# returaj/gan_mpc

Hardware: AMD Instinct MI355X
Metric: trajectories/sec (rollout+backward+critic step) at batch=1024, H=50 (higher is better)
Workload: dtype f32

## Files before the change

### gan_mpc_amd/csrc/gmpc_api_solve.hip

```cpp
#include "gmpc_ctx.h"
#include "gmpc_fused_solve.h"

static TrajArgs base_traj(gmpc_ctx* c, int B, const float* goal) {
  TrajArgs a;
  memset(&a, 0, sizeof(a));
  a.B = B; a.n = c->sh.n; a.m = c->sh.m; a.T = c->sh.T;
  a.dyn = c->dyn; a.cost = c->cost; a.mpc_w = c->mpc_w; a.goal = goal;
  return a;
}

static DynlTrajArgs base_dynl(gmpc_ctx* c, int B, const float* goal) {
  DynlTrajArgs a;
  memset(&a, 0, sizeof(a));
  a.B = B; a.T = c->sh.T; a.d = c->dl; a.cost = c->cost; a.mpc_w = c->mpc_w; a.goal = goal;
  return a;
}

extern "C" int gmpc_rollout_cost(gmpc_ctx* c, int B, const float* x0, const float* U,
                                 const float* goal, float* X, float* costs, void* stream) {
  TRY(check_call(c, B));
  if (!x0 || !U || !goal || !X) return fail(GMPC_EINVAL, "null argument");
  hipStream_t s = static_cast<hipStream_t>(stream);
  c->solB = 0;
  c->gradB = 0;
  if (c->dynl) {
    DynlTrajArgs d = base_dynl(c, B, goal);
    d.x0 = x0; d.U = U; d.X = X; d.costs = costs; d.obj = c->obj;
    {
      ProfScope ps(c, PROF_ROLLOUT, s);
      gmpc_launch_dynl_rollout(d, s);
    }
    HIP_TRY(hipGetLastError());
    return 0;
  }
  TrajArgs a = base_traj(c, B, goal);
  a.x0 = x0; a.U = U; a.X = X; a.costs = costs; a.obj = c->obj; a.masks = c->masks;
  {
    ProfScope ps(c, PROF_ROLLOUT, s);
    gmpc_launch_rollout(a, s);
  }
  HIP_TRY(hipGetLastError());
  return 0;
}

static int backward_pass(gmpc_ctx* c, int B, const float* X, const float* U, const float* goal,
                         const int* active, float* K, float* k, float* grad, float* adj, float* AB,
                         int* cont, const gmpc_ilqr_opts* opts, hipStream_t s) {
  const gmpc_shape& sh = c->sh;
  if (c->big) {
    if (c->lin_event) HIP_TRY(hipEventRecord(c->lin_event, s));
    if (gmpc_launch_terminal(B, sh.T, sh.n, c->cost, c->mpc_w, X, active, c->QT, c->qT, s) != 0)
      return fail(GMPC_EINVAL, "terminal: unsupported fout");
    HIP_TRY(hipGetLastError());
    {
      ProfScope ps(c, PROF_RICCATI, s);
      if (gmpc_big_backward(c->bw, B, c->dyn, c->lp, c->masks, X, U, goal, c->mpc_w, c->QT, c->qT, active,
                            c->Ks, k, grad ? grad : c->grads, adj ? adj : c->adjs, nullptr, nullptr, s,
                            c->dynl ? &c->dl : nullptr) != 0)
        return fail(GMPC_EINVAL, "large-state backward: Jacobian kernel does not cover this shape");
      if (K != c->Ks)
        HIP_TRY(hipMemcpyAsync(K, c->Ks, (size_t)B * sh.T * sh.m * sh.n * sizeof(float),
                               hipMemcpyDeviceToDevice, s));
    }
    if (cont)
      gmpc_launch_big_cont(B, sh.T, sh.m, U, c->bw.gn2, c->iters, c->obj, c->alpha, c->obj_step,
                           c->U_step, *opts, active, cont, s);
    HIP_TRY(hipGetLastError());
    return 0;
  }
  {
    ProfScope ps(c, PROF_TERMINAL, s);
    if (gmpc_launch_terminal(B, sh.T, sh.n, c->cost, c->mpc_w, X, active, c->QT, c->qT, s) != 0)
      return fail(GMPC_EINVAL, "terminal: unsupported fout");
  }
  {
    ProfScope ps(c, PROF_LINEARIZE, s);
    const char* lin_env = getenv("GMPC_LIN");
    const bool lin_dense = lin_env != nullptr && strcmp(lin_env, "dense") == 0;
    if (c->dynl) {
      gmpc_launch_dynl_jac(B, sh.T, sh.T, 0, c->dl, X, U, active, AB, s);
      c->lin_kernel = "k_dynl_jac";
    } else if (!lin_dense && gmpc_launch_linearize_sparse(B * sh.T, sh.T, sh.n, sh.m, c->dyn, c->lp, c->masks,
                                                          active, AB, 1, 0, s) == 0) {
      c->lin_kernel = sh.n > 16 ? "k_linearize_sparse (rows 0..15) + k_linearize_regs (rows 16..n-1)"
                                : "k_linearize_sparse";
    } else if (gmpc_launch_linearize_regs(B * sh.T, sh.T, sh.n, sh.m, c->dyn, c->lp, c->masks, active, AB, 1, 0,
                                          s) == 0) {
      snprintf(c->lin_kernel_buf, sizeof(c->lin_kernel_buf), "%s", gmpc_linearize_regs_last_name());
      c->lin_kernel = c->lin_kernel_buf;
    } else if (gmpc_launch_linearize_mfma(B * sh.T, sh.T, sh.n, sh.m, c->dyn, c->lp, c->masks, active, AB, 1, 0,
                                          s) != 0) {
      if (gmpc_launch_linearize(B, sh.T, sh.n, sh.m, c->dyn, c->masks, active, AB, s) != 0)
        return fail(GMPC_EINVAL, "linearize: unsupported row count for n=%d", sh.n);
      c->lin_kernel = "k_linearize (vector ALU)";
    } else {
      c->lin_kernel = "k_linearize_mfma";
    }
  }
  HIP_TRY(hipGetLastError());
  if (c->lin_event) HIP_TRY(hipEventRecord(c->lin_event, s));
  RiccatiArgs r;
  memset(&r, 0, sizeof(r));
  r.B = B; r.n = sh.n; r.ng = c->nx; r.m = sh.m; r.T = sh.T; r.mode = 0;
  r.X = X; r.U = U; r.goal = goal; r.mpc_w = c->mpc_w; r.AB = AB; r.QT = c->QT; r.qT = c->qT;
  r.active = active; r.K = K; r.k = k; r.grad = grad; r.adj = adj;
  if (cont) {
    r.cont = cont; r.iters = c->iters; r.obj = c->obj; r.alpha = c->alpha;
    r.obj_step = c->obj_step; r.U_step = c->U_step; r.opts = *opts;
  }
  {
    ProfScope ps(c, PROF_RICCATI, s);
    gmpc_launch_riccati(r, s);
  }
  HIP_TRY(hipGetLastError());
  return 0;
}

extern "C" int gmpc_lqr_backward(gmpc_ctx* c, int B, const float* X, const float* U,
                                 const float* goal, float* K, float* k, float* grad,
                                 float* adjoints, float* AB, void* stream) {
  TRY(check_call(c, B));
  if (!X || !U || !goal) return fail(GMPC_EINVAL, "null argument");
  hipStream_t s = static_cast<hipStream_t>(stream);
  if (c->big && AB) return fail(GMPC_EINVAL, "AB output is not materialised for n > 64 (pass NULL)");
  c->solB = 0;
  c->gradB = 0;
  if (!c->dynl) gmpc_launch_masks(B, c->sh.n, c->sh.m, c->sh.T, c->dyn, X, U, c->masks, s);
  return backward_pass(c, B, X, U, goal, nullptr, K ? K : c->Ks, k ? k : c->ks, grad, adjoints,
                       AB ? AB : c->AB, nullptr, nullptr, s);
}

extern "C" int gmpc_lqr_backward_after_rollout(gmpc_ctx* c, int B, const float* X, const float* U,
                                               const float* goal, float* K, float* k, float* grad,
                                               float* adjoints, float* AB, void* stream) {
  TRY(check_call(c, B));
  if (!X || !U || !goal) return fail(GMPC_EINVAL, "null argument");
  if (c->big && AB) return fail(GMPC_EINVAL, "AB output is not materialised for n > 64 (pass NULL)");
  hipStream_t s = static_cast<hipStream_t>(stream);
  c->solB = 0;
  c->gradB = 0;
  return backward_pass(c, B, X, U, goal, nullptr, K ? K : c->Ks, k ? k : c->ks, grad, adjoints,
                       AB ? AB : c->AB, nullptr, nullptr, s);
}

static void dynl_ls_eval(void* user, const TrajArgs& t, int max_items, hipStream_t s) {
  gmpc_ctx* c = static_cast<gmpc_ctx*>(user);
  DynlTrajArgs d = base_dynl(c, t.B, t.goal);
  d.item_b = t.item_b; d.item_k = t.item_k; d.nitems = t.nitems;
  d.Xn = t.X; d.Un = t.Uio; d.Kg = t.Kg; d.kg = t.kg;
  d.Xc = t.Xc; d.Uc = t.Uc; d.objc = t.objc; d.alpha_0 = t.alpha_0;
  gmpc_launch_dynl_candidates(d, max_items, s);
}

extern "C" int gmpc_ilqr_solve(gmpc_ctx* c, int B, const float* x0, const float* U_init,
                               const float* goal, const gmpc_ilqr_opts* opts, float* X, float* U,
                               float* obj, float* grad, float* adjoints, int* iterations,
                               void* stream) {
  TRY(check_call(c, B));
  if (!x0 || !U_init || !goal || !opts) return fail(GMPC_EINVAL, "null argument");
  if (opts->make_psd) return fail(GMPC_EINVAL, "make_psd=1 is not on the reference path");
  hipStream_t s = static_cast<hipStream_t>(stream);
  c->solB = 0;
  c->solBox = false;
  c->gradB = 0;
  const gmpc_shape& sh = c->sh;
  const size_t n = sh.n, m = sh.m, T = sh.T;
  HIP_TRY(hipMemcpyAsync(c->Us, U_init, B * T * m * sizeof(float), hipMemcpyDeviceToDevice, s));
  HIP_TRY(hipMemcpyAsync(c->goals, goal, B * (T + 1) * (size_t)c->nx * sizeof(float), hipMemcpyDeviceToDevice, s));
  HIP_TRY(hipMemsetAsync(c->iters, 0, B * sizeof(int), s));
  std::vector<float> init(3 * (size_t)B);
  for (int b = 0; b < B; ++b) {
    init[b] = opts->alpha_0;
    init[B + b] = INFINITY;
    init[2 * (size_t)B + b] = INFINITY;
  }
  HIP_TRY(hipMemcpyAsync(c->alpha, init.data(), B * sizeof(float), hipMemcpyHostToDevice, s));
  HIP_TRY(hipMemcpyAsync(c->obj_step, init.data() + B, B * sizeof(float), hipMemcpyHostToDevice, s));
  HIP_TRY(hipMemcpyAsync(c->U_step, init.data() + 2 * (size_t)B, B * sizeof(float),
                         hipMemcpyHostToDevice, s));
  HIP_TRY(hipStreamSynchronize(s));
  if (c->dynl) {
    DynlTrajArgs d = base_dynl(c, B, c->goals);
    d.x0 = x0; d.U = c->Us; d.X = c->Xs; d.costs = nullptr; d.obj = c->obj;
    gmpc_launch_dynl_rollout(d, s);
  } else {
    TrajArgs a = base_traj(c, B, c->goals);
    a.x0 = x0; a.U = c->Us; a.X = c->Xs; a.costs = nullptr; a.obj = c->obj; a.masks = c->masks;
    gmpc_launch_rollout(a, s);
  }
  TRY(backward_pass(c, B, c->Xs, c->Us, c->goals, nullptr, c->Ks, c->ks, c->grads, c->adjs, c->AB,
                    c->cont, opts, s));
  TrajArgs ls = base_traj(c, B, c->goals);
  ls.X = c->Xs; ls.Uio = c->Us; ls.obj = c->obj; ls.masks = c->masks; ls.Kg = c->Ks; ls.kg = c->ks;
  ls.Xc = c->Xc; ls.Uc = c->Uc; ls.maskc = c->maskc; ls.active = c->cont; ls.alpha = c->alpha;
  ls.obj_step = c->obj_step; ls.U_step = c->U_step; ls.iters = c->iters;
  ls.alpha_0 = opts->alpha_0; ls.alpha_min = opts->alpha_min;
  LsPlan plan;
  if (gmpc_ls_plan(ls, c->ncu, c->dynl, &plan) != 0 && opts->maxiter > 0)
    return fail(GMPC_EINVAL, "line search: alpha_0 / alpha_min need more than %d rounds", GMPC_LS_ROUNDS_MAX);
  HIP_TRY(hipMemsetAsync(c->lsw.prevk, 0, B * sizeof(int), s));
  HIP_TRY(hipMemsetAsync(c->lsw.counts + GMPC_LS_ROUNDS_MAX, 0, (1 + GMPC_LS_STATS) * sizeof(int), s));
  if (!c->hcont) {
    HIP_TRY(hipHostMalloc(reinterpret_cast<void**>(&c->hcont), (size_t)GMPC_POLL_DEPTH * c->maxB * sizeof(int),
                          hipHostMallocDefault));
    for (int i = 0; i < GMPC_POLL_DEPTH; ++i) HIP_TRY(hipEventCreateWithFlags(&c->poll_ev[i], hipEventDisableTiming));
  }
  for (int it = 0; it < opts->maxiter; ++it) {
    const int slot = it % GMPC_POLL_DEPTH;
    int* hc = c->hcont + (size_t)slot * c->maxB;
    if (it >= GMPC_POLL_DEPTH) {
      HIP_TRY(hipEventSynchronize(c->poll_ev[slot]));
      bool any = false;
      for (int b = 0; b < B; ++b) any |= hc[b] != 0;
      if (!any) break;
    }
    HIP_TRY(hipMemcpyAsync(hc, c->cont, B * sizeof(int), hipMemcpyDeviceToHost, s));
    HIP_TRY(hipEventRecord(c->poll_ev[slot], s));
    {
      ProfScope ps(c, PROF_LINESEARCH, s);
      gmpc_launch_linesearch(ls, plan, c->lsw, s, c->dynl ? &dynl_ls_eval : nullptr, c);
    }
    TRY(backward_pass(c, B, c->Xs, c->Us, c->goals, c->cont, c->Ks, c->ks, c->grads, c->adjs, c->AB,
                      c->cont, opts, s));
  }
  if (X) HIP_TRY(hipMemcpyAsync(X, c->Xs, B * (T + 1) * n * sizeof(float), hipMemcpyDeviceToDevice, s));
  if (U) HIP_TRY(hipMemcpyAsync(U, c->Us, B * T * m * sizeof(float), hipMemcpyDeviceToDevice, s));
  if (obj) HIP_TRY(hipMemcpyAsync(obj, c->obj, B * sizeof(float), hipMemcpyDeviceToDevice, s));
  if (grad) HIP_TRY(hipMemcpyAsync(grad, c->grads, B * T * m * sizeof(float), hipMemcpyDeviceToDevice, s));
  if (adjoints)
    HIP_TRY(hipMemcpyAsync(adjoints, c->adjs, B * (T + 1) * n * sizeof(float), hipMemcpyDeviceToDevice, s));
  if (iterations)
    HIP_TRY(hipMemcpyAsync(iterations, c->iters, B * sizeof(int), hipMemcpyDeviceToDevice, s));
  HIP_TRY(hipStreamSynchronize(s));
  c->solB = B;
  return 0;
}

static int solve_one_launch(gmpc_ctx* c, int B, const float* x0, const float* U_init, const float* goal,
                            const gmpc_ilqr_opts* opts, float* X, float* U, float* obj, float* grad, float* adjoints,
                            int* iterations, void* stream, const char* who, bool box, const float* u_lo,
                            const float* u_hi) {
  TRY(check_call(c, B));
  if (!x0 || !U_init || !goal || !opts) return fail(GMPC_EINVAL, "null argument");
  if (opts->make_psd) return fail(GMPC_EINVAL, "make_psd=1 is not on the reference path");
  const gmpc_shape& sh = c->sh;
  if (c->dynl) return fail(GMPC_EINVAL, "%s: MLP dynamics only (dyn_lstm_features = %d)", who, sh.dyn_lstm_features);
  if (c->big)
    return fail(GMPC_EINVAL, "%s: n <= 64 and m <= 32 only (n=%d m=%d)", who, sh.n, sh.m);
  if (sh.T > GMPC_FZ_MAX_T) return fail(GMPC_EINVAL, "%s: T <= %d only (T=%d)", who, GMPC_FZ_MAX_T, sh.T);
  const int k_max = gmpc_ls_halvings(opts->alpha_0, opts->alpha_min, GMPC_FZ_MAX_HALVINGS + 1);
  if (k_max > GMPC_FZ_MAX_HALVINGS)
    return fail(GMPC_EINVAL, "%s: alpha_0 / alpha_min allow more than %d halvings", who, GMPC_FZ_MAX_HALVINGS);
  hipStream_t s = static_cast<hipStream_t>(stream);
  c->solB = 0;
  c->solBox = false;
  c->gradB = 0;
  FusedSolveArgs a;
  memset(&a, 0, sizeof(a));
  a.n = sh.n; a.m = sh.m; a.T = sh.T; a.k_max = k_max;
  a.dyn = c->dyn; a.cost = c->cost; a.mpc_w = c->mpc_w; a.opts = *opts;
  a.x0 = x0; a.U_init = U_init; a.goal_in = goal;
  a.X = c->Xs; a.U = c->Us; a.goal = c->goals; a.AB = c->AB; a.QT = c->QT; a.qT = c->qT;
  a.K = c->Ks; a.k = c->ks; a.grad = c->grads; a.adj = c->adjs;
  a.obj = c->obj; a.alpha = c->alpha; a.obj_step = c->obj_step; a.U_step = c->U_step; a.iters = c->iters;
  a.cand = c->fzcand;
  a.oX = X; a.oU = U; a.oobj = obj; a.ograd = grad; a.oadj = adjoints; a.oiters = iterations;
  if (box) {
    BoxSolveArgs x;
    x.u_lo = u_lo; x.u_hi = u_hi;
    x.count = c->box_count; x.iters = c->box_iters; x.clamped = c->box_clamped;
    gmpc_launch_ilqr_box(a, x, B, s);
  } else {
    gmpc_launch_ilqr_fused(a, B, s);
  }
  HIP_TRY(hipGetLastError());
  return 0;
}

extern "C" int gmpc_ilqr_solve_fused(gmpc_ctx* c, int B, const float* x0, const float* U_init,
                                     const float* goal, const gmpc_ilqr_opts* opts, float* X, float* U,
                                     float* obj, float* grad, float* adjoints, int* iterations,
                                     void* stream) {
  TRY(solve_one_launch(c, B, x0, U_init, goal, opts, X, U, obj, grad, adjoints, iterations, stream, "fused solve",
                       false, nullptr, nullptr));
  c->solB = B;
  return 0;
}

extern "C" int gmpc_ilqr_solve_box(gmpc_ctx* c, int B, const float* x0, const float* U_init,
                                   const float* goal, const gmpc_ilqr_opts* opts, float* X, float* U,
                                   float* obj, float* grad, float* adjoints, int* iterations,
                                   void* stream, const float* u_lo, const float* u_hi) {
  return solve_one_launch(c, B, x0, U_init, goal, opts, X, U, obj, grad, adjoints, iterations, stream, "box solve",
                          true, u_lo, u_hi);
}

extern "C" int gmpc_ilqr_solve_box_held(gmpc_ctx* c, int B, const float* x0, const float* U_init,
                                        const float* goal, const gmpc_ilqr_opts* opts, float* X, float* U,
                                        float* obj, float* grad, float* adjoints, int* iterations,
                                        void* stream, const float* u_lo, const float* u_hi) {
  TRY(solve_one_launch(c, B, x0, U_init, goal, opts, X, U, obj, grad, adjoints, iterations, stream, "box solve",
                       true, u_lo, u_hi));
  gmpc_launch_box_clamped(B, c->sh.T, c->sh.m, c->Us, c->grads, u_lo, u_hi, c->box_mask,
                          static_cast<hipStream_t>(stream));
  HIP_TRY(hipGetLastError());
  c->solB = B;
  c->solBox = true;
  return 0;
}

extern "C" int gmpc_cem_solve(gmpc_ctx* c, int B, const float* x0, const float* goal, const float* u_lo,
                              const float* u_hi, const gmpc_cem_opts* o, float* mean_io, float* std_io, float* X,
                              float* obj, float* costs, int* elites, float* samples, void* stream) {
  TRY(check_call(c, B));
  const gmpc_shape& sh = c->sh;
  if (c->dynl) return fail(GMPC_EINVAL, "cem: MLP dynamics only (dyn_lstm_features = %d)", sh.dyn_lstm_features);
  for (int l = 0; l <= sh.dyn_layers; ++l)
    if (sh.dyn_dims[l] > 256) return fail(GMPC_EINVAL, "cem: dynamics width %d above 256", sh.dyn_dims[l]);
  for (int l = 0; l <= sh.cost_layers; ++l)
    if (sh.cost_dims[l] > 256) return fail(GMPC_EINVAL, "cem: cost width %d above 256", sh.cost_dims[l]);
  if (sh.n + sh.m > 256) return fail(GMPC_EINVAL, "cem: n + m = %d above 256", sh.n + sh.m);
  if (!o) return fail(GMPC_EINVAL, "cem: opts is null");
  if (!x0 || !goal || !mean_io || !std_io) return fail(GMPC_EINVAL, "cem: x0, goal, mean_io and std_io must not be null");
  if (o->num_samples < 1 || o->num_samples > 4096)
    return fail(GMPC_EINVAL, "cem: num_samples = %d outside [1, 4096]", o->num_samples);
  if (o->num_elites < 1 || o->num_elites > o->num_samples)
    return fail(GMPC_EINVAL, "cem: num_elites = %d outside [1, num_samples = %d]", o->num_elites, o->num_samples);
  if (o->max_iter < 0) return fail(GMPC_EINVAL, "cem: max_iter = %d is negative", o->max_iter);
  if (!(o->sampling_smoothing >= 0.f && o->sampling_smoothing < 1.f))
    return fail(GMPC_EINVAL, "cem: sampling_smoothing = %g outside [0, 1)", (double)o->sampling_smoothing);
  if (!(o->evolution_smoothing >= 0.f && o->evolution_smoothing <= 1.f))
    return fail(GMPC_EINVAL, "cem: evolution_smoothing = %g outside [0, 1]", (double)o->evolution_smoothing);
  hipStream_t s = static_cast<hipStream_t>(stream);
  const int N = o->num_samples;
  float* cost_buf = costs;
  if (!cost_buf && o->max_iter > 0) {
    TRY(c->cw.aux.grow(c, (size_t)B * N));
    cost_buf = c->cw.aux.p;
  }
  CemRollArgs r;
  memset(&r, 0, sizeof(r));
  r.B = B; r.N = N; r.T = sh.T; r.n = sh.n; r.m = sh.m;
  r.dyn = c->dyn; r.cost = c->cost; r.mpc_w = c->mpc_w;
  r.x0 = x0; r.goal = goal; r.mean = mean_io; r.sd = std_io; r.lo = u_lo; r.hi = u_hi;
  r.rng.key0 = (uint32_t)(o->seed & 0xFFFFFFFFull); r.rng.key1 = (uint32_t)(o->seed >> 32);
  r.rng.beta = o->sampling_smoothing;
  r.rng.cbeta = sqrtf(1.f - r.rng.beta * r.rng.beta);
  r.costs = cost_buf;
  CemUpdArgs u;
  memset(&u, 0, sizeof(u));
  u.B = B; u.N = N; u.E = o->num_elites; u.T = sh.T; u.m = sh.m;
  u.costs = cost_buf; u.lo = u_lo; u.hi = u_hi; u.mean = mean_io; u.sd = std_io;
  u.gamma = o->evolution_smoothing;
  for (int i = 0; i < o->max_iter; ++i) {
    const bool last = i == o->max_iter - 1;
    r.rng.it = (uint32_t)(o->iter_offset + i);
    r.samples = last ? samples : nullptr;
    u.rng = r.rng;
    u.elites = last ? elites : nullptr;
    if (gmpc_launch_cem_rollout(r, s) || gmpc_launch_cem_update(u, s)) return fail(GMPC_EINVAL, "cem: shape not covered");
  }
  if (X || obj) {
    if (!obj) {
      TRY(c->cw.aux2.grow(c, (size_t)B));
      obj = c->cw.aux2.p;
    }
    r.N = 1; r.mean_row = 1; r.samples = nullptr; r.costs = obj; r.X = X;
    if (gmpc_launch_cem_rollout(r, s)) return fail(GMPC_EINVAL, "cem: shape not covered");
  }
  HIP_TRY(hipGetLastError());
  return 0;
}


extern "C" int gmpc_get_cost(gmpc_ctx* c, int B, const float* x, const float* u, const float* goal_row,
                             int terminal, float* cost, void* stream) {
  TRY(check_call(c, B));
  if (!x || !cost || (!terminal && (!u || !goal_row))) return fail(GMPC_EINVAL, "null argument");
  gmpc_launch_get_cost(B, c->sh.n, c->nx, c->sh.m, c->cost, c->mpc_w, x, u, goal_row, terminal != 0, cost,
                       static_cast<hipStream_t>(stream));
  HIP_TRY(hipGetLastError());
  return 0;
}

extern "C" int gmpc_predict(gmpc_ctx* c, int B, const float* x, const float* u, float* next_x,
                            void* stream) {
  TRY(check_call(c, B));
  if (!x || !u || !next_x) return fail(GMPC_EINVAL, "null argument");
  hipStream_t s = static_cast<hipStream_t>(stream);
  const size_t n = c->sh.n;
  c->solB = 0;
  c->gradB = 0;
  HIP_TRY(hipMemsetAsync(c->goals, 0, (size_t)B * 2 * n * sizeof(float), s));
  if (c->dynl) {
    DynlTrajArgs d = base_dynl(c, B, c->goals);
    d.T = 1;
    d.x0 = x; d.U = u; d.X = c->Xc; d.costs = nullptr; d.obj = c->obj;
    gmpc_launch_dynl_rollout(d, s);
  } else {
    TrajArgs a = base_traj(c, B, c->goals);
    a.T = 1;
    a.x0 = x; a.U = u; a.X = c->Xc; a.costs = nullptr; a.obj = c->obj; a.masks = c->masks;
    gmpc_launch_rollout(a, s);
  }
  HIP_TRY(hipGetLastError());
  HIP_TRY(hipMemcpy2DAsync(next_x, n * sizeof(float), c->Xc + n, 2 * n * sizeof(float), n * sizeof(float),
                           B, hipMemcpyDeviceToDevice, s));
  return 0;
}

extern "C" long gmpc_linesearch_candidates(gmpc_ctx* c) {
  if (!c) return -1;
  int v = 0;
  if (hipSetDevice(c->device) != hipSuccess || hipDeviceSynchronize() != hipSuccess ||
      hipMemcpy(&v, c->lsw.counts + GMPC_LS_ROUNDS_MAX, sizeof(int), hipMemcpyDeviceToHost) != hipSuccess)
    return -1;
  return v;
}

extern "C" int gmpc_linesearch_stats(gmpc_ctx* c, long* out, int n) {
  if (!c || !out) return fail(GMPC_EINVAL, "ctx / out is null");
  int v[GMPC_LS_STATS];
  HIP_TRY(hipSetDevice(c->device));
  HIP_TRY(hipDeviceSynchronize());
  HIP_TRY(hipMemcpy(v, c->lsw.counts + GMPC_LS_ROUNDS_MAX + 1, sizeof(v), hipMemcpyDeviceToHost));
  for (int i = 0; i < n; ++i) out[i] = i < GMPC_LS_STATS ? v[i] : 0;
  return 0;
}
```

### gan_mpc_amd/csrc/gmpc_linearize_sparse.hip

```cpp
#include <cstdio>
#include <type_traits>

#include "gmpc_launch.h"

typedef float f32x4 __attribute__((ext_vector_type(4)));
typedef unsigned v4u __attribute__((ext_vector_type(4)));
typedef unsigned v2u __attribute__((ext_vector_type(2)));

#define GMPC_LIN_PADROWS 24
#define GMPC_SP_H 200
#define GMPC_SP_Z 200
#define GMPC_SP_STR 220
#define GMPC_SP_CAP 216
#define GMPC_SP_WAVE_BYTES (16 * GMPC_SP_STR * 4 + 3 * GMPC_SP_CAP * 4)
#define GMPC_SP_RD 3
#define GMPC_SP_ROW 256

static bool sparse_form(int L, const int* dims, int n, int m) {
  const int Lh = L - 1;
  if (Lh < 2 || n + m > 32 || n < 1) return false;
  for (int l = 1; l <= Lh; ++l)
    if (dims[l] != GMPC_SP_H) return false;
  return true;
}

__global__ void k_pack_sparse(const float* W, float* dst) {
  const int e = blockIdx.x * blockDim.x + threadIdx.x;
  if (e >= GMPC_SP_H * GMPC_SP_H) return;
  const int i = e / GMPC_SP_H, o = e - i * GMPC_SP_H;
  const int t = i >> 4;
  const int slot = i < 192 ? 64 * (t >> 2) + 4 * (i & 15) + (t & 3) : i;
  dst[(size_t)o * GMPC_SP_ROW + slot] = W[e];
}

size_t gmpc_linsparse_floats(int L, const int* dims, int n, int m) {
  if (!sparse_form(L, dims, n, m)) return 0;
  return (size_t)(L - 2) * (GMPC_SP_H + GMPC_LIN_PADROWS) * GMPC_SP_ROW + GMPC_SP_ROW;
}

void gmpc_linsparse_prepare(const MlpDesc& dyn, int n, int m, float* p, LinPad* out, hipStream_t s) {
  for (int l = 0; l < GMPC_MAX_LAYERS; ++l) out->WSP[l] = nullptr;
  if (!sparse_form(dyn.L, dyn.dims, n, m)) return;
  p = reinterpret_cast<float*>((reinterpret_cast<uintptr_t>(p) + 1023) & ~(uintptr_t)1023);
  for (int l = 1; l < dyn.L - 1; ++l) {
    out->WSP[l] = p;
    hipLaunchKernelGGL(k_pack_sparse, dim3((GMPC_SP_H * GMPC_SP_H + 255) / 256), dim3(256), 0, s, dyn.W[l], p);
    p += (size_t)(GMPC_SP_H + GMPC_LIN_PADROWS) * GMPC_SP_ROW;
  }
}

__global__ __launch_bounds__(GMPC_THREADS, 2) void k_linearize_sparse(
    int NSamp, int T, int n, int m, int Lh, LinPad lp, const uint32_t* masks, const int* active, float* AB,
    int samp_mul, int samp_add) {
  extern __shared__ __attribute__((aligned(16))) char smem[];
  const int lane = threadIdx.x & 63, wave = __builtin_amdgcn_readfirstlane(threadIdx.x >> 6);
  const int g = lane >> 4, l16 = lane & 15;
  const int nm = n + m;
  const int nrow = n < 16 ? n : 16;
  char* wbase = smem + wave * GMPC_SP_WAVE_BYTES;
  float* st = reinterpret_cast<float*>(wbase);
  unsigned* lk = reinterpret_cast<unsigned*>(wbase + 16 * GMPC_SP_STR * 4);
  unsigned* lt = lk + GMPC_SP_CAP;
  if (lane < 16 * 8) st[(lane >> 3) * GMPC_SP_STR + GMPC_SP_H + (lane & 7)] = 0.f;
  if (lane + 64 < 16 * 8) st[((lane + 64) >> 3) * GMPC_SP_STR + GMPC_SP_H + (lane & 7)] = 0.f;

  const int lw = l16 * 16, lwt = (192 + (l16 & 7)) * 4;
  const int ls = l16 * GMPC_SP_STR * 4;
  const int tsel = l16 >= 8 ? 1 : 0;
  const unsigned* lkl = lk + g;
  const unsigned* ltl_ = lt + 2 * g + tsel;
  const int lsn = l16 < n ? l16 * 4 : (1 << 28);
  const __amdgpu_buffer_rsrc_t rsl = __builtin_amdgcn_make_buffer_rsrc(
      const_cast<float*>(lp.WLP), 0, (GMPC_SP_H + GMPC_LIN_PADROWS) * n * (int)sizeof(float), 0x00020000);
  const __amdgpu_buffer_rsrc_t rs0 = __builtin_amdgcn_make_buffer_rsrc(
      const_cast<float*>(lp.WTP[0]), 0, (GMPC_SP_H + GMPC_LIN_PADROWS) * 32 * (int)sizeof(float), 0x00020000);

  constexpr int WPB = GMPC_THREADS / 64;
  for (int s = blockIdx.x * WPB + wave; s < NSamp; s += gridDim.x * WPB) {
    const size_t sid = (size_t)s * samp_mul + samp_add;
    if (active != nullptr && active[sid / T] == 0) continue;
    const uint32_t* mrow = masks + sid * Lh * GMPC_MW;

    auto build = [&](int ml) -> int {
      __builtin_amdgcn_wave_barrier();
      int base = 0;
#pragma unroll
      for (int c = 0; c < 4; ++c) {
        const uint32_t lo = __builtin_amdgcn_readfirstlane(mrow[ml * GMPC_MW + 2 * c]);
        uint32_t hi = c < 3 ? __builtin_amdgcn_readfirstlane(mrow[ml * GMPC_MW + 2 * c + 1]) : 0u;
        const uint32_t lo_m = c < 3 ? lo : (lo & 0xFFu);
        const uint32_t word = lane < 32 ? lo_m : hi;
        const int pos = base + (int)__builtin_amdgcn_mbcnt_hi(hi, __builtin_amdgcn_mbcnt_lo(lo_m, 0u));
        const unsigned u = 64 * c + lane;
        if ((word >> (lane & 31)) & 1u) {
          const bool odd = (u & 1u) != 0;
          lk[pos] = u;
          *reinterpret_cast<v2u*>(lt + 2 * pos) = v2u{odd ? GMPC_SP_Z : u, odd ? u : GMPC_SP_Z};
        }
        base += __builtin_popcount(lo_m) + __builtin_popcount(hi);
      }
      if (lane < 16) {
        lk[base + lane] = GMPC_SP_Z;
        *reinterpret_cast<v2u*>(lt + 2 * (base + lane)) = v2u{GMPC_SP_Z, GMPC_SP_Z};
      }
      __builtin_amdgcn_wave_barrier();
      return base;
    };

    auto layer = [&](int l, auto seedc) __attribute__((always_inline)) {
      constexpr bool seed = decltype(seedc)::value;
      const int np = (build(l) + 3) >> 2;
      const __amdgpu_buffer_rsrc_t wrs = __builtin_amdgcn_make_buffer_rsrc(
          const_cast<float*>(lp.WSP[l]), 0, (GMPC_SP_H + GMPC_LIN_PADROWS) * GMPC_SP_ROW * 4, 0x00020000);
      f32x4 acc[13];
      struct Ops { float w[13]; float b; unsigned k, kt; };
      Ops r[GMPC_SP_RD];
      auto tables = [&](Ops& o, int p) {
        o.k = lkl[4 * p];
        o.kt = ltl_[8 * p];
      };
      auto loads = [&](Ops& o) {
        const int k = (int)o.k, kt = (int)o.kt;
        const int vo = (k << 10) + lw, vt = (kt << 10) + lwt;
#pragma unroll
        for (int q = 0; q < 3; ++q) {
          const v4u a = __builtin_amdgcn_raw_buffer_load_b128(wrs, vo + 256 * q, 0, 0);
          o.w[4 * q] = __uint_as_float(a.x); o.w[4 * q + 1] = __uint_as_float(a.y);
          o.w[4 * q + 2] = __uint_as_float(a.z); o.w[4 * q + 3] = __uint_as_float(a.w);
        }
        o.w[12] = __uint_as_float(__builtin_amdgcn_raw_buffer_load_b32(wrs, vt, 0, 0));
        if constexpr (seed) o.b = __uint_as_float(__builtin_amdgcn_raw_buffer_load_b32(rsl, k * n * 4 + lsn, 0, 0));
        else o.b = st[(ls >> 2) + k];
      };
      auto step = [&](int p, Ops& cur, Ops& ahead2) __attribute__((always_inline)) {
        loads(ahead2);
        tables(cur, p + 3);
        __builtin_amdgcn_sched_barrier(0);
#pragma unroll
        for (int t = 0; t < 13; ++t) acc[t] = __builtin_amdgcn_mfma_f32_16x16x4f32(cur.w[t], cur.b, acc[t], 0, 0, 0);
        __builtin_amdgcn_sched_barrier(0);
      };
      if (np == 0) {
#pragma unroll
        for (int t = 0; t < 13; ++t) acc[t] = f32x4{0.f, 0.f, 0.f, 0.f};
      } else {
        tables(r[0], 0); tables(r[1], 1); tables(r[2], 2);
        loads(r[0]); loads(r[1]);
        loads(r[2]);
        tables(r[0], 3);
        __builtin_amdgcn_sched_barrier(0);
#pragma unroll
        for (int t = 0; t < 13; ++t)
          acc[t] = __builtin_amdgcn_mfma_f32_16x16x4f32(r[0].w[t], r[0].b, f32x4{0.f, 0.f, 0.f, 0.f}, 0, 0, 0);
        __builtin_amdgcn_sched_barrier(0);
        int p = 1;
        for (; p + 3 <= np; p += 3) {
          step(p, r[1], r[0]);
          step(p + 1, r[2], r[1]);
          step(p + 2, r[0], r[2]);
        }
        if (p < np) step(p, r[1], r[0]);
        if (p + 1 < np) step(p + 1, r[2], r[1]);
      }
      mfma_fence<false>(acc[0], acc[1], acc[2], acc[3], acc[4], acc[5], acc[6], acc[7], acc[8], acc[9], acc[10],
                        acc[11], acc[12]);
      __builtin_amdgcn_wave_barrier();
      float* srow = st + l16 * GMPC_SP_STR;
#pragma unroll
      for (int t = 0; t < 12; ++t)
        *reinterpret_cast<f32x4*>(srow + 32 * (t >> 1) + 16 * (t & 1) + 4 * g) = acc[t];
      *reinterpret_cast<f32x4*>(srow + (g < 2 ? 192 : 200) + 4 * g) = acc[12];
      __builtin_amdgcn_wave_barrier();
      if (g < 2) {
        const f32x4 x = *reinterpret_cast<const f32x4*>(srow + 192 + 4 * g);
        const f32x4 y = *reinterpret_cast<const f32x4*>(srow + 208 + 4 * g);
        *reinterpret_cast<f32x4*>(srow + 192 + 4 * g) = x + y;
      }
      __builtin_amdgcn_wave_barrier();
    };
    layer(Lh - 1, std::true_type{});
    for (int l = Lh - 2; l >= 1; --l) layer(l, std::false_type{});

    {
      const int np = (build(0) + 3) >> 2;
      f32x4 acc0 = {0.f, 0.f, 0.f, 0.f}, acc1 = {0.f, 0.f, 0.f, 0.f};
      const bool two = nm > 16;
      struct Ops0 { float w0, w1, b; unsigned k; };
      Ops0 r[GMPC_SP_RD];
      auto tables = [&](Ops0& o, int p) { o.k = lkl[4 * p]; };
      auto loads = [&](Ops0& o) {
        const int vo = (int)(o.k << 7) + l16 * 4;
        o.w0 = __uint_as_float(__builtin_amdgcn_raw_buffer_load_b32(rs0, vo, 0, 0));
        o.w1 = __uint_as_float(__builtin_amdgcn_raw_buffer_load_b32(rs0, vo + 64, 0, 0));
        o.b = st[(ls >> 2) + o.k];
      };
      auto step = [&](int p, Ops0& cur, Ops0& ahead2) __attribute__((always_inline)) {
        loads(ahead2);
        tables(cur, p + 3);
        __builtin_amdgcn_sched_barrier(0);
        acc0 = __builtin_amdgcn_mfma_f32_16x16x4f32(cur.w0, cur.b, acc0, 0, 0, 0);
        acc1 = __builtin_amdgcn_mfma_f32_16x16x4f32(cur.w1, cur.b, acc1, 0, 0, 0);
        __builtin_amdgcn_sched_barrier(0);
      };
      tables(r[0], 0); tables(r[1], 1); tables(r[2], 2);
      loads(r[0]); loads(r[1]);
      int p = 0;
      for (; p + 3 <= np; p += 3) {
        step(p, r[0], r[2]);
        step(p + 1, r[1], r[0]);
        step(p + 2, r[2], r[1]);
      }
      if (p < np) step(p, r[0], r[2]);
      if (p + 1 < np) step(p + 1, r[1], r[0]);
      mfma_fence<false>(acc0, acc1);
      if (l16 < nrow) {
        float* dst = AB + ((size_t)s * n + l16) * nm;
#pragma unroll
        for (int j = 0; j < 4; ++j) {
          const int c = 4 * g + j;
          if (c < nm) dst[c] = acc0[j] + (c == l16 ? 1.0f : 0.0f);
          if (two && c + 16 < nm) dst[c + 16] = acc1[j] + (c + 16 == l16 ? 1.0f : 0.0f);
        }
      }
    }
    __builtin_amdgcn_wave_barrier();
  }
}

int gmpc_launch_linearize_sparse(int NSamp, int T, int n, int m, const MlpDesc& dyn, const LinPad& lp,
                                 const uint32_t* masks, const int* active, float* AB, int samp_mul, int samp_add,
                                 hipStream_t s) {
  const int Lh = dyn.L - 1;
  if (!sparse_form(dyn.L, dyn.dims, n, m) || lp.NT != 7 || lp.NTF != 1 || lp.NGF != 1) return -1;
  if (NSamp <= 0) return 0;
  if (n > 16 && gmpc_launch_linearize_regs_rows(NSamp, T, n, m, dyn, lp, masks, active, AB, samp_mul, samp_add, 16,
                                                s) != 0)
    return -1;
  const size_t lds = (size_t)(GMPC_THREADS / 64) * GMPC_SP_WAVE_BYTES;
  int grid = (NSamp + 3) / 4;
  if (grid > 256 * 2) grid = 256 * 2;
  hipLaunchKernelGGL(k_linearize_sparse, dim3(grid), dim3(GMPC_THREADS), lds, s, NSamp, T, n, m, Lh, lp, masks,
                     active, AB, samp_mul, samp_add);
  return 0;
}
```

Before: 802,200.

## Compute Jacobian rows 16..n-1 in sparse kernel by grouping 16 time samples per wave

When n>16 and samples are contiguous, the separate k_linearize_regs launch for rows 16..n-1 is dropped. Each wave instead takes a contiguous chunk of samples and, for each extra output row, processes up to 16 samples together. The wave builds a union sparsity list across those samples and masks per-sample activations with keep_if bit-extracts, so a single MFMA sweep serves 16 samples. This is meant to remove a kernel launch and the slower register path, at the cost of wasted work where the samples' masks differ and more complex control flow.

```diff
diff --git a/gan_mpc_amd/csrc/gmpc_api_solve.hip b/gan_mpc_amd/csrc/gmpc_api_solve.hip
--- a/gan_mpc_amd/csrc/gmpc_api_solve.hip
+++ b/gan_mpc_amd/csrc/gmpc_api_solve.hip
@@ -82,7 +82,7 @@
       c->lin_kernel = "k_dynl_jac";
     } else if (!lin_dense && gmpc_launch_linearize_sparse(B * sh.T, sh.T, sh.n, sh.m, c->dyn, c->lp, c->masks,
                                                           active, AB, 1, 0, s) == 0) {
-      c->lin_kernel = sh.n > 16 ? "k_linearize_sparse (rows 0..15) + k_linearize_regs (rows 16..n-1)"
+      c->lin_kernel = sh.n > 16 ? "k_linearize_sparse (rows 0..15 per sample, rows 16..n-1 per time group)"
                                 : "k_linearize_sparse";
     } else if (gmpc_launch_linearize_regs(B * sh.T, sh.T, sh.n, sh.m, c->dyn, c->lp, c->masks, active, AB, 1, 0,
                                           s) == 0) {
diff --git a/gan_mpc_amd/csrc/gmpc_linearize_sparse.hip b/gan_mpc_amd/csrc/gmpc_linearize_sparse.hip
--- a/gan_mpc_amd/csrc/gmpc_linearize_sparse.hip
+++ b/gan_mpc_amd/csrc/gmpc_linearize_sparse.hip
@@ -1,5 +1,6 @@
 #include <cstdio>
 #include <type_traits>
+#include <utility>
 
 #include "gmpc_launch.h"
 
@@ -49,9 +50,24 @@
   }
 }
 
+template <int BIT>
+__device__ __forceinline__ float keep_if(float v, uint32_t w) {
+  unsigned full, vb = __float_as_uint(v);
+  asm("v_bfe_i32 %1, %2, %3, 1\n\tv_and_b32 %0, %0, %1" : "+v"(vb), "=&v"(full) : "v"(w), "n"(BIT));
+  return __uint_as_float(vb);
+}
+template <int... J>
+__device__ __forceinline__ f32x4 keep_if4(f32x4 v, uint32_t w, std::integer_sequence<int, J...>) {
+  return f32x4{keep_if<J>(v[J & 3], w)...};
+}
+template <int B0>
+__device__ __forceinline__ f32x4 keep_if4(f32x4 v, uint32_t w) {
+  return keep_if4(v, w, std::integer_sequence<int, B0, B0 + 1, B0 + 2, B0 + 3>{});
+}
+
 __global__ __launch_bounds__(GMPC_THREADS, 2) void k_linearize_sparse(
     int NSamp, int T, int n, int m, int Lh, LinPad lp, const uint32_t* masks, const int* active, float* AB,
-    int samp_mul, int samp_add) {
+    int samp_mul, int samp_add, int grouped) {
   extern __shared__ __attribute__((aligned(16))) char smem[];
   const int lane = threadIdx.x & 63, wave = __builtin_amdgcn_readfirstlane(threadIdx.x >> 6);
   const int g = lane >> 4, l16 = lane & 15;
@@ -75,19 +91,49 @@
   const __amdgpu_buffer_rsrc_t rs0 = __builtin_amdgcn_make_buffer_rsrc(
       const_cast<float*>(lp.WTP[0]), 0, (GMPC_SP_H + GMPC_LIN_PADROWS) * 32 * (int)sizeof(float), 0x00020000);
 
-  constexpr int WPB = GMPC_THREADS / 64;
-  for (int s = blockIdx.x * WPB + wave; s < NSamp; s += gridDim.x * WPB) {
-    const size_t sid = (size_t)s * samp_mul + samp_add;
-    if (active != nullptr && active[sid / T] == 0) continue;
+  auto job = [&](auto grpc, int s, int jr, int cnt) __attribute__((always_inline)) {
+    constexpr bool GRP = decltype(grpc)::value;
+    bool cvalid = true;
+    size_t sid = (size_t)s * samp_mul + samp_add;
+    if constexpr (GRP) {
+      cvalid = l16 < cnt;
+      if (cvalid) sid = (size_t)s + l16;
+      if (cvalid && active != nullptr) cvalid = active[sid / T] != 0;
+      if (__ballot(cvalid) == 0ull) return;
+    } else {
+      if (active != nullptr && active[sid / T] == 0) return;
+    }
     const uint32_t* mrow = masks + sid * Lh * GMPC_MW;
 
+    auto colwords = [&](int ml, uint32_t (&w)[7]) {
+#pragma unroll
+      for (int i = 0; i < 7; ++i) w[i] = cvalid ? mrow[ml * GMPC_MW + i] : 0u;
+      w[6] &= 0xFFu;
+    };
+    auto listwords = [&](int ml, uint32_t (&w)[7]) {
+      if constexpr (GRP) {
+        colwords(ml, w);
+#pragma unroll
+        for (int i = 0; i < 7; ++i) {
+#pragma unroll
+          for (int d = 1; d < 16; d <<= 1) w[i] |= (uint32_t)__shfl_xor((int)w[i], d);
+          w[i] = __builtin_amdgcn_readfirstlane(w[i]);
+        }
+      } else {
+#pragma unroll
+        for (int i = 0; i < 7; ++i) w[i] = __builtin_amdgcn_readfirstlane(mrow[ml * GMPC_MW + i]);
+      }
+    };
+
     auto build = [&](int ml) -> int {
       __builtin_amdgcn_wave_barrier();
+      uint32_t mw[7];
+      listwords(ml, mw);
       int base = 0;
 #pragma unroll
       for (int c = 0; c < 4; ++c) {
-        const uint32_t lo = __builtin_amdgcn_readfirstlane(mrow[ml * GMPC_MW + 2 * c]);
-        uint32_t hi = c < 3 ? __builtin_amdgcn_readfirstlane(mrow[ml * GMPC_MW + 2 * c + 1]) : 0u;
+        const uint32_t lo = mw[2 * c];
+        uint32_t hi = c < 3 ? mw[2 * c + 1] : 0u;
         const uint32_t lo_m = c < 3 ? lo : (lo & 0xFFu);
         const uint32_t word = lane < 32 ? lo_m : hi;
         const int pos = base + (int)__builtin_amdgcn_mbcnt_hi(hi, __builtin_amdgcn_mbcnt_lo(lo_m, 0u));
@@ -113,6 +159,13 @@
       const __amdgpu_buffer_rsrc_t wrs = __builtin_amdgcn_make_buffer_rsrc(
           const_cast<float*>(lp.WSP[l]), 0, (GMPC_SP_H + GMPC_LIN_PADROWS) * GMPC_SP_ROW * 4, 0x00020000);
       f32x4 acc[13];
+      uint32_t cw[7];
+      if constexpr (GRP) {
+        colwords(l - 1, cw);
+#pragma unroll
+        for (int i = 0; i < 6; ++i) cw[i] >>= 4 * g;
+        cw[6] >>= 4 * (g & 1);
+      }
       struct Ops { float w[13]; float b; unsigned k, kt; };
       Ops r[GMPC_SP_RD];
       auto tables = [&](Ops& o, int p) {
@@ -165,6 +218,15 @@
       mfma_fence<false>(acc[0], acc[1], acc[2], acc[3], acc[4], acc[5], acc[6], acc[7], acc[8], acc[9], acc[10],
                         acc[11], acc[12]);
       __builtin_amdgcn_wave_barrier();
+      if constexpr (GRP) {
+        acc[0] = keep_if4<0>(acc[0], cw[0]); acc[1] = keep_if4<16>(acc[1], cw[0]);
+        acc[2] = keep_if4<0>(acc[2], cw[1]); acc[3] = keep_if4<16>(acc[3], cw[1]);
+        acc[4] = keep_if4<0>(acc[4], cw[2]); acc[5] = keep_if4<16>(acc[5], cw[2]);
+        acc[6] = keep_if4<0>(acc[6], cw[3]); acc[7] = keep_if4<16>(acc[7], cw[3]);
+        acc[8] = keep_if4<0>(acc[8], cw[4]); acc[9] = keep_if4<16>(acc[9], cw[4]);
+        acc[10] = keep_if4<0>(acc[10], cw[5]); acc[11] = keep_if4<16>(acc[11], cw[5]);
+        acc[12] = keep_if4<0>(acc[12], cw[6]);
+      }
       float* srow = st + l16 * GMPC_SP_STR;
 #pragma unroll
       for (int t = 0; t < 12; ++t)
@@ -178,8 +240,37 @@
       }
       __builtin_amdgcn_wave_barrier();
     };
-    layer(Lh - 1, std::true_type{});
-    for (int l = Lh - 2; l >= 1; --l) layer(l, std::false_type{});
+    if constexpr (GRP) {
+      __builtin_amdgcn_wave_barrier();
+      float* srow = st + l16 * GMPC_SP_STR + 4 * g;
+      const uint32_t* mcol = mrow + (Lh - 1) * GMPC_MW;
+      const int wo = (4 * g * n + jr) * 4;
+#pragma unroll 1
+      for (int nt = 0; nt < 6; ++nt) {
+        const uint32_t cw = (cvalid ? mcol[nt] : 0u) >> (4 * g);
+        f32x4 v0, v1;
+#pragma unroll
+        for (int j = 0; j < 4; ++j) {
+          v0[j] = __uint_as_float(__builtin_amdgcn_raw_buffer_load_b32(rsl, wo + (32 * nt + j) * n * 4, 0, 0));
+          v1[j] = __uint_as_float(__builtin_amdgcn_raw_buffer_load_b32(rsl, wo + (32 * nt + 16 + j) * n * 4, 0, 0));
+        }
+        *reinterpret_cast<f32x4*>(srow + 32 * nt) = keep_if4<0>(v0, cw);
+        *reinterpret_cast<f32x4*>(srow + 32 * nt + 16) = keep_if4<16>(v1, cw);
+      }
+      if (g < 2) {
+        const uint32_t cw = (cvalid ? mcol[6] & 0xFFu : 0u) >> (4 * g);
+        f32x4 v;
+#pragma unroll
+        for (int j = 0; j < 4; ++j)
+          v[j] = __uint_as_float(__builtin_amdgcn_raw_buffer_load_b32(rsl, wo + (192 + j) * n * 4, 0, 0));
+        *reinterpret_cast<f32x4*>(srow + 192) = keep_if4<0>(v, cw);
+      }
+      __builtin_amdgcn_wave_barrier();
+      for (int l = Lh - 1; l >= 1; --l) layer(l, std::false_type{});
+    } else {
+      layer(Lh - 1, std::true_type{});
+      for (int l = Lh - 2; l >= 1; --l) layer(l, std::false_type{});
+    }
 
     {
       const int np = (build(0) + 3) >> 2;
@@ -213,17 +304,38 @@
       if (p < np) step(p, r[0], r[2]);
       if (p + 1 < np) step(p + 1, r[1], r[0]);
       mfma_fence<false>(acc0, acc1);
-      if (l16 < nrow) {
-        float* dst = AB + ((size_t)s * n + l16) * nm;
+      const int orow = GRP ? jr : l16;
+      if (GRP ? cvalid : l16 < nrow) {
+        float* dst = AB + ((size_t)(GRP ? s + l16 : s) * n + orow) * nm;
 #pragma unroll
         for (int j = 0; j < 4; ++j) {
           const int c = 4 * g + j;
-          if (c < nm) dst[c] = acc0[j] + (c == l16 ? 1.0f : 0.0f);
-          if (two && c + 16 < nm) dst[c + 16] = acc1[j] + (c + 16 == l16 ? 1.0f : 0.0f);
+          if (c < nm) dst[c] = acc0[j] + (c == orow ? 1.0f : 0.0f);
+          if (two && c + 16 < nm) dst[c + 16] = acc1[j] + (c + 16 == orow ? 1.0f : 0.0f);
         }
       }
     }
     __builtin_amdgcn_wave_barrier();
+  };
+
+  constexpr int WPB = GMPC_THREADS / 64;
+  const int w = blockIdx.x * WPB + wave, W = gridDim.x * WPB;
+  if (!grouped) {
+    for (int s = w; s < NSamp; s += W) job(std::false_type{}, s, 0, 0);
+    return;
+  }
+  const int C = (NSamp + W - 1) / W;
+  const long c0l = (long)w * C;
+  const int c0 = c0l < NSamp ? (int)c0l : NSamp;
+  const int len = NSamp - c0 < C ? NSamp - c0 : C;
+  for (int s = c0; s < c0 + len; ++s) job(std::false_type{}, s, 0, 0);
+  if (n > 16 && len > 0) {
+    const int ng = (len + 15) >> 4;
+    for (int r = 16; r < n; ++r)
+      for (int i = 0; i < ng; ++i) {
+        const int a = i * len / ng, b = (i + 1) * len / ng;
+        job(std::true_type{}, c0 + a, r, b - a);
+      }
   }
 }
 
@@ -233,13 +345,14 @@
   const int Lh = dyn.L - 1;
   if (!sparse_form(dyn.L, dyn.dims, n, m) || lp.NT != 7 || lp.NTF != 1 || lp.NGF != 1) return -1;
   if (NSamp <= 0) return 0;
-  if (n > 16 && gmpc_launch_linearize_regs_rows(NSamp, T, n, m, dyn, lp, masks, active, AB, samp_mul, samp_add, 16,
-                                                s) != 0)
+  const int grouped = samp_mul == 1 && samp_add == 0;
+  if (n > 16 && !grouped &&
+      gmpc_launch_linearize_regs_rows(NSamp, T, n, m, dyn, lp, masks, active, AB, samp_mul, samp_add, 16, s) != 0)
     return -1;
   const size_t lds = (size_t)(GMPC_THREADS / 64) * GMPC_SP_WAVE_BYTES;
   int grid = (NSamp + 3) / 4;
   if (grid > 256 * 2) grid = 256 * 2;
   hipLaunchKernelGGL(k_linearize_sparse, dim3(grid), dim3(GMPC_THREADS), lds, s, NSamp, T, n, m, Lh, lp, masks,
-                     active, AB, samp_mul, samp_add);
+                     active, AB, samp_mul, samp_add, grouped);
   return 0;
 }
```

New measurement: 840,100, median of 6. +4.7%, better.
